# EdwardLiuyc/StaticMapping

Measured on AMD Instinct MI355X. Metric: scan-pair alignments/sec (120k-pt KITTI-64, 20 ICP iters), higher is better.
Workload: dtype f32/f64; 1 GPU; BASELINE config #2: IcpFast point-to-plane, 120k-pt synthetic Velodyne-64 scan pair vs CalculateNormals target (~21695 pts), exactly 20 iterations, rho 0.7; 512 distinct consecutive pairs of a synthetic drive (speed 6-10 m/s, yaw rate +-0.2 rad/s, seed 5), guess = previous pair's motion; pairs_per_gpu=512, distinct_pairs=512, target_points_mean=21695, nn_mode=grid, guess=extrapolated, split_after=2, parallelism=pairs round-robin over 1 GPU(s), one RCCL gather of poses, rccl_ranks=1

## Files before the change

### staticmapping_amd/csrc/icp_kernels.hip

```cpp
#include <type_traits>
#include "smhip_device.h"
#include "kd_median_tree.h"
#include "grid_lookup.h"

namespace smhip {

__device__ __forceinline__ bool xcd_block(int nblk, int npairs, int b_pair_base, int& pair, int& blk) {
  const int id = blockIdx.x;
  const int j = id >> 3;
  const int local = (j / nblk) * 8 + (id & 7);
  pair = b_pair_base + local;
  blk = j % nblk;
  return local < npairs;
}

__global__ __launch_bounds__(256) void tgt_reduce(IcpDev b) {
  const int pair = b.pair_base + blockIdx.y;
  const int nt = b.in[pair].nt;
  const float4* tp = b.tgt_p + (size_t)pair * b.nt_cap;
  double sx = 0, sy = 0, sz = 0;
  float mn[3] = {INFINITY, INFINITY, INFINITY}, mx[3] = {-INFINITY, -INFINITY, -INFINITY};
  const int chunk = (nt + gridDim.x - 1) / gridDim.x;
  const int lo = blockIdx.x * chunk, hi = min(nt, lo + chunk);
  for (int j = lo + threadIdx.x; j < hi; j += blockDim.x) {
// ... 1711 lines not shown
  if (threadIdx.x == 0) {
    const uint32_t active = (uint32_t)((nt + per - 1) / per);
    s_last = atomicAdd(&st->fallback_ticket, 1u) == active - 1u ? 1u : 0u;
  }
  __syncthreads();
  if (!s_last) return;
  __threadfence();
  for (int e = threadIdx.x; e < U; e += kNnThreads) {
    const int i = b.ulist[so + e];
    const unsigned long long key = __hip_atomic_load(&b.ukeys[so + e], __ATOMIC_RELAXED, __HIP_MEMORY_SCOPE_AGENT);
    const uint32_t dbits = (uint32_t)(key >> 32);
    b.d2[so + i] = __uint_as_float(dbits);
    st_match(b, so + i, (int)(uint32_t)(key & 0xffffffffu), 0.f);
    if (dbits < 0x7f800000u) atomicAdd(&b.hist[(size_t)pair * kHistBins + (dbits >> kHistShift)], 1u);
  }
  if (threadIdx.x == 0) st->fallback_ticket = 0;
}
__global__ __launch_bounds__(kNnThreads) void nn_fallback(IcpDev b) {
  const int pair = b.pair_base + blockIdx.y;
  PairState* st = &b.state[pair];
  if (st->done) return;
  __shared__ float4 s_t[kBruteTile];
  __shared__ uint32_t s_last;
  fallback_body(b, st, pair, (int)blockIdx.x, (int)gridDim.x, s_t, &s_last);
}


__device__ __forceinline__ int quantile_rank(uint32_t n_valid, float rho) {
  const double q = (double)rho;
  if (q >= 1.0) return (int)n_valid - 1;
  int k = (int)((double)n_valid * q);
  return min(k, (int)n_valid - 1);
}

__device__ __forceinline__ void find_quantile_bin_counts(const uint32_t* c, float rho, uint32_t* s_w, uint32_t* s_out) {
  constexpr int per = kHistBins / 256;
  uint32_t sum = 0;
#pragma unroll
  for (int k = 0; k < per; ++k) sum += c[k];
  uint32_t total;
  const uint32_t excl = block_excl_scan(sum, s_w, &total);
  if (threadIdx.x == 0) { s_out[0] = 0xffffffffu; s_out[1] = 0; s_out[2] = total; s_out[3] = 0; }
  __syncthreads();
  if (total > 0) {
    const uint32_t k = (uint32_t)quantile_rank(total, rho);
    if (excl <= k && k < excl + sum) {
      uint32_t run = excl;
#pragma unroll
      for (int t = 0; t < per; ++t) {
        if (k < run + c[t]) { s_out[0] = threadIdx.x * per + t; s_out[1] = run; s_out[3] = k; break; }
        run += c[t];
      }
    }
  }
  __syncthreads();
}
__device__ __forceinline__ void find_quantile_bin(const uint32_t* __restrict__ gh, float rho, uint32_t* s_w, uint32_t* s_out) {
  constexpr int per = kHistBins / 256;
  uint32_t c[per];
#pragma unroll
  for (int k = 0; k < per; ++k) c[k] = gh[threadIdx.x * per + k];
  find_quantile_bin_counts(c, rho, s_w, s_out);
}

__device__ __forceinline__ void validate_bounds(const IcpDev& b, PairState* st, int pair, uint32_t* s_w, uint32_t* s_q) {
  find_quantile_bin(b.hist + (size_t)pair * kHistBins, b.rho, s_w, s_q);
  if (threadIdx.x == 0) {
    const bool any = st->hard_count > 0;
    const bool below = (st->min_lb_key >> kHistShift) <= s_q[0];
    st->refine = (any && (b.exact_all || below || s_q[2] == 0)) ? 1 : 0;
    if (st->refine) st->refine_total += 1;
    st->spec_ok = (b.fused && st->band_lo > 0 && !st->refine && s_q[2] > 0 && (int)s_q[0] >= st->band_lo && (int)s_q[0] <= st->band_hi &&
                   st->deferred_count <= (uint32_t)kFusedListedMax) ? 1 : 0;
  }
}

__global__ __launch_bounds__(256) void nn_validate(IcpDev b) {
  const int pair = b.pair_base + blockIdx.x;
  PairState* st = &b.state[pair];
  if (st->done) return;
  __shared__ uint32_t s_w[17];
  __shared__ uint32_t s_q[4];
  validate_bounds(b, st, pair, s_w, s_q);
}

__global__ __launch_bounds__(kNnThreads) void nn_refine_one(IcpDev b) {
  const int pair = b.pair_base + blockIdx.x;
  PairState* st = &b.state[pair];
  if (st->done) return;
  __shared__ uint32_t s_w[17];
  __shared__ uint32_t s_q[4];
  __shared__ uint32_t s_hist[kHistBins];
  __shared__ float4 s_t[kBruteTile];
  __shared__ uint32_t s_last;
  validate_bounds(b, st, pair, s_w, s_q);
  __syncthreads();
  if (!st->refine) return;
  ring_body<true>(b, st, pair, 0, 1, s_hist);
  __syncthreads();
  fallback_body(b, st, pair, 0, 1, s_t, &s_last);
}

template <bool COUNT = true>
__device__ __forceinline__ void accumulate_terms_p(double px, double py, double pz, const float4 q4, const float4 n4, double* acc) {
  const double nx = n4.x, ny = n4.y, nz = n4.z;
  double J[6];
  J[0] = py * nz - pz * ny;
  J[1] = pz * nx - px * nz;
  J[2] = px * ny - py * nx;
  J[3] = nx; J[4] = ny; J[5] = nz;
  const double r = (px - (double)q4.x) * nx + (py - (double)q4.y) * ny + (pz - (double)q4.z) * nz;
  int c = 0;
#pragma unroll
  for (int a = 0; a < 6; ++a)
#pragma unroll
    for (int e = a; e < 6; ++e) acc[c++] += J[a] * J[e];
#pragma unroll
  for (int a = 0; a < 6; ++a) acc[21 + a] += J[a] * r;
  if (COUNT) acc[28] += 1.0;
}
__device__ __forceinline__ void accumulate_terms(const double* M, const float4 s4, const float4 q4, const float4 n4, double* acc) {
  double px, py, pz;
  transform_point(M, s4, px, py, pz);
  accumulate_terms_p(px, py, pz, q4, n4, acc);
}
template <int CTRL, int ROW_MASK>
__device__ __forceinline__ double dpp_or_zero(double v) {
  const int lo = __builtin_amdgcn_update_dpp(0, __double2loint(v), CTRL, ROW_MASK, 0xf, false);
  const int hi = __builtin_amdgcn_update_dpp(0, __double2hiint(v), CTRL, ROW_MASK, 0xf, false);
  return __hiloint2double(hi, lo);
}
__device__ __forceinline__ double wave_sum_to_last(double v) {
  v += dpp_or_zero<0x111, 0xf>(v);
  v += dpp_or_zero<0x112, 0xf>(v);
  v += dpp_or_zero<0x114, 0xf>(v);
  v += dpp_or_zero<0x118, 0xf>(v);
  v += dpp_or_zero<0x142, 0xa>(v);
  v += dpp_or_zero<0x143, 0xc>(v);
  return v;
}

__device__ __forceinline__ void block_reduce29(double* acc, double (*s_red)[29], double* s_out) {
  const int lane = threadIdx.x & 63, wave = threadIdx.x >> 6;
#pragma unroll
  for (int c = 0; c < 29; ++c) acc[c] = wave_sum_to_last(acc[c]);
  if (lane == 63)
#pragma unroll
    for (int c = 0; c < 29; ++c) s_red[wave][c] = acc[c];
  __syncthreads();
  if (threadIdx.x < 29) s_out[threadIdx.x] = ((s_red[0][threadIdx.x] + s_red[1][threadIdx.x]) + s_red[2][threadIdx.x]) + s_red[3][threadIdx.x];
  __syncthreads();
}

template <int ITEMS>
__device__ __forceinline__ void accumulate_block(const IcpDev& b, PairState* st, int pair, int blk, const double* Mc,
                                                 uint32_t* s_w, uint32_t* s_q, double (*s_red)[29], double* s_out) {
  const int ns = st->ns;
  const int base = blk * (kAccThreads * ITEMS);
  find_quantile_bin(b.hist + (size_t)pair * kHistBins, b.rho, s_w, s_q);
  const uint32_t qbin = s_q[0];
  double acc[29];
#pragma unroll
  for (int c = 0; c < 29; ++c) acc[c] = 0.0;
  const size_t so = (size_t)pair * b.ns_cap;
  const size_t to = (size_t)pair * b.nt_cap;
  const int seg = blk * (kAccThreads / 64) + (int)(threadIdx.x >> 6);
  const size_t segbase = (size_t)pair * 2 * b.bl_stride + (size_t)seg * (64 * ITEMS);
  int wcount = 0;
  int ic = min(base + (int)threadIdx.x, ns - 1);
  float d_1 = b.d2[so + ic];
  float4 s_1 = ld_src(b, so + ic);
  int j_1 = b.idx[so + ic];
  ic = min(base + kAccThreads + (int)threadIdx.x, ns - 1);
  float d_2 = b.d2[so + ic];
  float4 s_2 = ld_src(b, so + ic);
  int j_2 = b.idx[so + ic];
  float4 q_1 = make_float4(0, 0, 0, 0), n_1 = make_float4(0, 0, 0, 0);
  if ((__float_as_uint(d_1) >> kHistShift) < qbin) { q_1 = b.tq[to + max(j_1, 0)]; n_1 = b.tn[to + max(j_1, 0)]; }
#pragma unroll 2
  for (int it = 0; it < ITEMS; ++it) {
    const int i = base + it * kAccThreads + threadIdx.x;
    const float d = d_1;
    const float4 s4 = s_1;
    const float4 q4 = q_1, n4 = n_1;
    const int jm = j_1;
    d_1 = d_2; s_1 = s_2; j_1 = j_2;
    if (it + 1 < ITEMS && (__float_as_uint(d_1) >> kHistShift) < qbin) { q_1 = b.tq[to + max(j_1, 0)]; n_1 = b.tn[to + max(j_1, 0)]; }
    if (it + 2 < ITEMS) {
      ic = min(i + 2 * kAccThreads, ns - 1);
      d_2 = b.d2[so + ic];
      s_2 = ld_src(b, so + ic);
      j_2 = b.idx[so + ic];
    }
    bool boundary = false;
    if (i < ns) {
      const uint32_t key = __float_as_uint(d);
      if (key < 0x7f800000u) {
        const uint32_t bin = key >> kHistShift;
        if (bin < qbin) accumulate_terms(Mc, s4, q4, n4, acc);
        else boundary = bin == qbin;
      }
    }
    const unsigned long long bm = __ballot(boundary);
    if (boundary) {
      const size_t at = segbase + wcount + __popcll(bm & ((1ull << (threadIdx.x & 63)) - 1ull));
      b.rec_a[at] = make_float4(s4.x, s4.y, s4.z, d);
      b.rec_j[at] = jm;
    }
    wcount += (int)__popcll(bm);
  }
  if ((threadIdx.x & 63) == 0) b.gcount[(size_t)pair * b.seg_stride + seg] = (uint32_t)wcount;
  block_reduce29(acc, s_red, s_out);
  if (threadIdx.x < 29) b.partials[((size_t)pair * b.part_stride + blk) * kAccCols + threadIdx.x] = s_out[threadIdx.x];
}

template <int ITEMS>
__global__ __launch_bounds__(kAccThreads) void accumulate(IcpDev b, int nblk) {
  int pair, blk;
  if (!xcd_block(nblk, b.npairs, b.pair_base, pair, blk)) return;
  PairState* st = &b.state[pair];
  if (st->done) return;
  if (b.fused && st->spec_ok) return;
  if (blk * (kAccThreads * ITEMS) >= st->ns) return;
  double Mc[12];
#pragma unroll
  for (int k = 0; k < 12; ++k) Mc[k] = st->M[k];
  __shared__ uint32_t s_w[17];
  __shared__ uint32_t s_q[4];
  __shared__ double s_red[4][29];
  __shared__ double s_out[29];
  accumulate_block<ITEMS>(b, st, pair, blk, Mc, s_w, s_q, s_red, s_out);
}


__device__ __forceinline__ uint32_t rank_below(unsigned long long mask) {
  return __builtin_amdgcn_mbcnt_hi((uint32_t)(mask >> 32), __builtin_amdgcn_mbcnt_lo((uint32_t)mask, 0u));
}
__device__ __forceinline__ void emit_record(const IcpDev& b, size_t segbase, int& wcount, bool band, unsigned long long bm, const float4 s, float d, int j) {
  if (band) {
    const uint32_t k = rank_below(bm);
    char* __restrict__ ra = reinterpret_cast<char*>(b.rec_a + segbase + wcount);
    char* __restrict__ rj = reinterpret_cast<char*>(b.rec_j + segbase + wcount);
    *reinterpret_cast<float4*>(ra + k * 16u) = make_float4(s.x, s.y, s.z, d);
    *reinterpret_cast<int32_t*>(rj + k * 4u) = j;
  }
  wcount += (int)__popcll(bm);
}

template <int ITEMS, bool NABO = false, bool SHADOW = false>
__global__ __launch_bounds__(kNnThreads, NABO ? 4 : 1) void nn_certify_acc(IcpDev b, int nblk) {
  int pair, blk;
  if (!xcd_block(nblk, b.npairs, b.pair_base, pair, blk)) return;
  PairState* st = &b.state[pair];
  if (st->done) return;
  const int ns = st->ns;
  const int base = blk * (kNnThreads * ITEMS);
  if (base >= ns) return;
  double Mc[12];
#pragma unroll
  for (int k = 0; k < 12; ++k) Mc[k] = st->M[k];
  asm volatile("" : "+v"(Mc[3]), "+v"(Mc[7]), "+v"(Mc[11]));
  const Pot pot = {(float)st->pot_a, (float)st->pot_b, 0.f, 0.f};
  const int band_lo = st->band_lo, band_hi = st->band_hi;
  __shared__ uint32_t s_hist[kHistBins];
  __shared__ double s_red[4][29];
  __shared__ double s_out[29];
  for (int k = threadIdx.x; k < kHistBins; k += kNnThreads) s_hist[k] = 0;
  __syncthreads();
  const int lane = threadIdx.x & 63;
  const size_t so = (size_t)pair * b.ns_cap, to = (size_t)pair * b.nt_cap;
  const char* __restrict__ tqb = reinterpret_cast<const char*>(b.tq + to);
  const char* __restrict__ tnb = reinterpret_cast<const char*>(b.tn + to);
  const char* __restrict__ srcb = reinterpret_cast<const char*>(b.src3 + 3 * so);
  const char* __restrict__ lbb = reinterpret_cast<const char*>(b.lb + so);
  const char* __restrict__ idxb = reinterpret_cast<const char*>(b.idx + so);
  const char* __restrict__ mbb = reinterpret_cast<const char*>(b.mb + so);
  char* __restrict__ d2b = reinterpret_cast<char*>(b.d2 + so);
  auto ld_s = [&](int k) { const float3 v = *reinterpret_cast<const float3*>(srcb + __umul24((uint32_t)k, 12u)); return make_float4(v.x, v.y, v.z, 0.f); };
  auto ld_l = [&](int k) { return *reinterpret_cast<const float*>(lbb + (uint32_t)k * 4u); };
  auto ld_j = [&](int k) { return *reinterpret_cast<const int*>(idxb + (uint32_t)k * 4u); };
  auto ld_m = [&](int k) { return *reinterpret_cast<const uint32_t*>(mbb + (uint32_t)k * 4u); };
  auto ld_t = [&](const char* base, int j) { const float3 v = *reinterpret_cast<const float3*>(base + (uint32_t)max(j, 0) * 16u); return make_float4(v.x, v.y, v.z, 0.f); };
  auto st_d = [&](int k, float v) { *reinterpret_cast<float*>(d2b + (uint32_t)k * 4u) = v; };
  const float r_need = 0.9f * sqrtf(st->rcap2);
  uint32_t min_lb = 0xffffffffu;
  const int seg = blk * (kNnThreads / 64) + __builtin_amdgcn_readfirstlane((int)(threadIdx.x >> 6));
  const size_t recbase = (size_t)pair * 2 * b.bl_stride + (size_t)seg * (64 * ITEMS);
  char* __restrict__ dsegb = reinterpret_cast<char*>(b.dlist + (size_t)pair * b.dl_stride + (size_t)seg * (64 * ITEMS));
  int nrec = 0, ndef = 0, nkept = 0;
  uint32_t nabo_failed = 0;
  double acc[29];
#pragma unroll
  for (int c = 0; c < 29; ++c) acc[c] = 0.0;
  int ic = min(base + (int)threadIdx.x, ns - 1);
  float4 s_1 = ld_s(ic);
  float l_1, l_2;
  int j_1, j_2;
  uint32_t m_2 = 0;
  if (SHADOW) { const uint32_t m = ld_m(ic); l_1 = shadow_bound(m); j_1 = shadow_match(m); }
  else { l_1 = ld_l(ic); j_1 = ld_j(ic); }
  ic = min(base + kNnThreads + (int)threadIdx.x, ns - 1);
  float4 s_2 = ld_s(ic);
  if (SHADOW) { m_2 = ld_m(ic); l_2 = 0.f; j_2 = 0; }
  else { l_2 = ld_l(ic); j_2 = ld_j(ic); }
  float4 t_1 = ld_t(tqb, j_1);
  float4 n_1 = ld_t(tnb, j_1);
  auto round = [&](const int it, auto GATHER, auto STREAM) {
    const int i = base + it * kNnThreads + threadIdx.x;
    bool hard = false, fail = false, band = false;
    const float4 s = s_1;
    const float l = l_1;
    const int j = j_1;
    const float4 t = t_1, n = n_1;
    s_1 = s_2;
    if (SHADOW) { l_1 = shadow_bound(m_2); j_1 = shadow_match(m_2); }
    else { l_1 = l_2; j_1 = j_2; }
    if (GATHER.value) { t_1 = ld_t(tqb, j_1); n_1 = ld_t(tnb, j_1); }
    if (STREAM.value) {
      ic = min(i + 2 * kNnThreads, ns - 1);
      s_2 = ld_s(ic);
      if (SHADOW) m_2 = ld_m(ic);
      else { l_2 = ld_l(ic); j_2 = ld_j(ic); }
    }
    float d1 = 0.f;
    unsigned long long m_fail = 0, m_band = 0, m_hard = 0;
    if (NABO) {
      bool keep = false;
      if (i < ns) {
        double px, py, pz;
        transform_point(Mc, s, px, py, pz);
        const float qx = (float)px, qy = (float)py, qz = (float)pz;
        fail = true;
        const float Pn = pot_at(pot, norm3(s.x, s.y, s.z));
        if (isfinite(qx) && isfinite(qy) && isfinite(qz) && l > 0.f && j >= 0 &&
            l - Pn - 4.0e-7f * (l + Pn) - 1.3e-7f * (fabsf(qx) + fabsf(qy) + fabsf(qz)) > 0.f) {
          d1 = dist2(t, qx, qy, qz);
          st_d(i, d1);
          const int bin = (int)(__float_as_uint(d1) >> kHistShift);
          atomicAdd(&s_hist[bin], 1u);
          fail = false;
          if (bin < band_lo) { accumulate_terms_p<false>(px, py, pz, t, n, acc); keep = true; }
          else band = bin <= band_hi;
        }
      }
      nkept += (int)__popcll(__ballot(keep));
    } else {
      const auto B = [](bool p) { return (unsigned long long)__builtin_amdgcn_ballot_w64(p); };
      const auto P = [](unsigned long long m) { return (bool)__builtin_amdgcn_inverse_ballot_w64(m); };
      double px, py, pz;
      transform_point(Mc, s, px, py, pz);
      const float qx = (float)px, qy = (float)py, qz = (float)pz;
      const float Lp = bound_now(l, pot_at(pot, __builtin_amdgcn_sqrtf(fmaf(s.z, s.z, fmaf(s.y, s.y, s.x * s.x)))));
      const unsigned long long m_inr = B(i < ns);
      const unsigned long long m_pos = m_inr & B(Lp > 0.f);
      const unsigned long long m_has = B(l > 0.f) & B(j >= 0);
      d1 = dist2(t, qx, qy, qz);
      const unsigned long long m_ok = m_pos & m_has & B(d1 < Lp * Lp);
      const float zq = fmaf(qz, 0.f, fmaf(qy, 0.f, qx * 0.f));
      m_hard = m_pos & B(zq == 0.f) & ~m_has & B(l < 0.f) & B(Lp >= r_need);
      m_fail = m_inr & ~(m_ok | m_hard);
      const int bin = (int)(__float_as_uint(d1) >> kHistShift);
      const unsigned long long m_keep = m_ok & B(bin < band_lo);
      m_band = m_ok & ~m_keep & B(bin <= band_hi);
      nkept += (int)__popcll(m_keep);
      fail = P(m_fail); band = P(m_band); hard = P(m_hard);
      if (P(m_ok)) {
        st_d(i, d1);
        atomicAdd(&s_hist[bin], 1u);
      }
      if (P(m_keep)) accumulate_terms_p<false>(px, py, pz, t, n, acc);
      if (hard) {
        const float lb2 = Lp * Lp;
        st_d(i, lb2);
        atomicAdd(&s_hist[__float_as_uint(lb2) >> kHistShift], 1u);
        min_lb = min(min_lb, __float_as_uint(lb2));
      }
    }
    if (NABO) {
      if (fail) nabo_failed |= 1u << it;
      m_band = __ballot(band);
    } else {
      if (fail) *reinterpret_cast<int*>(dsegb + ((uint32_t)ndef + rank_below(m_fail)) * 4u) = i;
      ndef += (int)__popcll(m_fail);
    }
    emit_record(b, recbase, nrec, band, m_band, s, d1, j);
    const unsigned long long hm = m_hard;
    if (hm) {
      uint32_t basepos = 0;
      if (lane == 0) basepos = atomicAdd(&st->hard_count, (uint32_t)__popcll(hm));
      basepos = (uint32_t)__builtin_amdgcn_readlane((int)basepos, 0);
      if (hard) b.hlist[so + basepos + __popcll(hm & ((1ull << lane) - 1ull))] = i;
    }
  };
  static_assert(ITEMS >= 2, "the pipeline's last two rounds are written out");
#pragma unroll 2
  for (int it = 0; it < ITEMS - 2; ++it) round(it, std::true_type{}, std::true_type{});
  round(ITEMS - 2, std::true_type{}, std::false_type{});
  round(ITEMS - 1, std::false_type{}, std::false_type{});
  if (lane == 0) {
    b.gcount[(size_t)pair * b.seg_stride + seg] = (uint32_t)nrec;
    b.dcount[(size_t)pair * b.seg_stride + seg] = ndef;
  }
#pragma unroll
  for (int off = 32; off > 0; off >>= 1) min_lb = min(min_lb, (uint32_t)__shfl_xor((int)min_lb, off, 64));
  if (lane == 0 && min_lb != 0xffffffffu) atomicMin(&st->min_lb_key, min_lb);
  if (lane == 0) acc[28] = (double)nkept;
  block_reduce29(acc, s_red, s_out);
  if (threadIdx.x < 29) b.partials[((size_t)pair * b.part_stride + blk) * kAccCols + threadIdx.x] = s_out[threadIdx.x];
  if (NABO) nabo_list_append<ITEMS>(b, st, so, base, ns, nabo_failed, lane);
  uint32_t* gh = b.hist + (size_t)pair * kHistBins;
  for (int k = threadIdx.x; k < kHistBins; k += kNnThreads) {
    const uint32_t v = s_hist[k];
    if (v) atomicAdd(&gh[k], v);
  }
}

struct ListedCtx {
  const uint2* __restrict__ words; const uint32_t* __restrict__ cstart; const float4* __restrict__ tq;
  float ox, oy, oz, h, inv_h, r2cap;
  int nx, ny, nz, wx;
  uint32_t nt_last;
  bool have_prev;
  Pot pot;
};
__device__ __forceinline__ ListedCtx listed_ctx(const IcpDev& b, const PairState* st, int pair) {
  ListedCtx c;
  c.words = b.words + (size_t)pair * kMaxGridWords;
  c.cstart = b.cstart + (size_t)pair * (b.nt_cap + 1);
  c.tq = b.tq + (size_t)pair * b.nt_cap;
  c.ox = st->origin[0]; c.oy = st->origin[1]; c.oz = st->origin[2];
  c.h = st->h; c.inv_h = st->inv_h; c.r2cap = st->rcap2;
  c.nx = st->nx; c.ny = st->ny; c.nz = st->nz; c.wx = st->wx;
  c.nt_last = (uint32_t)max(st->nt - 1, 0);
  c.have_prev = st->iter > 0;
  c.pot = {(float)st->pot_a, (float)st->pot_b, 0.f, 0.f};
  return c;
}
__device__ __forceinline__ void listed_search_one(const IcpDev& b, const PairState* st, const ListedCtx& c, size_t so, int i, int sub, int L,
                                                  uint32_t* s_hist, uint32_t& min_lb, bool& hard, bool track_band, int band_lo, int band_hi,
                                                  bool& band, float4& srec, float& drec, int& jrec) {
  if (i < 0) {
    return;
  }
  const float4 s4 = ld_src(b, so + i);
  double px, py, pz;
  transform_point(st->M, s4, px, py, pz);
  const float qx = (float)px, qy = (float)py, qz = (float)pz;
  Best best = {INFINITY, -1, INFINITY};
  const bool finite = isfinite(qx) && isfinite(qy) && isfinite(qz);
  float R2 = c.r2cap;
  int jp = -1;
  if (finite) {
    if (c.have_prev) {
      jp = b.idx[so + i];
      if (jp >= 0) {
        double ux, uy, uz;
        transform_point(st->M_prev, s4, ux, uy, uz);
        const float ex = qx - (float)ux, ey = qy - (float)uy, ez = qz - (float)uz;
        R2 = search_radius2(c.r2cap, dist2(c.tq[jp], qx, qy, qz), search_margin(sqrtf(fmaf(ez, ez, fmaf(ey, ey, ex * ex)))));
      }
    }
    const float Rs = sqrtf(R2) * 1.0001f + 1.0e-3f * c.h;
    const int x0 = max(cell_coord(qx - Rs, c.ox, c.inv_h), 0), x1 = min(cell_coord(qx + Rs, c.ox, c.inv_h), c.nx - 1);
    const int y0 = max(cell_coord(qy - Rs, c.oy, c.inv_h), 0), y1 = min(cell_coord(qy + Rs, c.oy, c.inv_h), c.ny - 1);
    const int z0 = max(cell_coord(qz - Rs, c.oz, c.inv_h), 0), z1 = min(cell_coord(qz + Rs, c.oz, c.inv_h), c.nz - 1);
    const int nyr = y1 - y0 + 1;
    const int nrows = (x0 <= x1 && y0 <= y1 && z0 <= z1) ? nyr * (z1 - z0 + 1) : 0;
    const float slack = 2.0e-3f * c.h;
    const float inv_nyr = 1.0f / (float)max(nyr, 1);
    const uint32_t wa_i = (uint32_t)(x0 >> 5), wc_i = (uint32_t)(x1 >> 5);
    const uint32_t ma = (1u << (x0 & 31)) - 1u, mc = 0xffffffffu >> (31 - (x1 & 31));
    for (int rb = sub; rb < nrows; rb += 4 * L) {
      bool ok[4];
      uint2 wa[4], wc[4];
#pragma unroll
      for (int k = 0; k < 4; ++k) {
        const int r = rb + k * L, rr = min(r, nrows - 1);
        const int zr = (int)(((float)rr + 0.5f) * inv_nyr);
        const int z = z0 + zr, y = y0 + (rr - zr * nyr);
        const float zl = c.oz + (float)z * c.h, yl = c.oy + (float)y * c.h;
        const float dz = fmaxf(fmaxf(zl - qz, qz - (zl + c.h)) - slack, 0.f);
        const float dy = fmaxf(fmaxf(yl - qy, qy - (yl + c.h)) - slack, 0.f);
        ok[k] = r < nrows && !(fmaf(dy, dy, dz * dz) > R2);
        const int rowbase = (z * c.ny + y) * c.wx;
        wa[k] = c.words[rowbase + wa_i];
        wc[k] = c.words[rowbase + wc_i];
      }
      uint32_t j0[4], j1[4];
#pragma unroll
      for (int k = 0; k < 4; ++k) {
        const uint32_t sb = wa[k].y + __popc(wa[k].x & ma), se = wc[k].y + __popc(wc[k].x & mc);
        const bool has = ok[k] && se > sb;
        j0[k] = c.cstart[has ? sb : 0u];
        j1[k] = c.cstart[has ? se : 0u];
      }
      float4 t0[4];
#pragma unroll
      for (int k = 0; k < 4; ++k) t0[k] = c.tq[min(j0[k], c.nt_last)];
#pragma unroll
      for (int k = 0; k < 4; ++k) {
        if (j1[k] > j0[k]) {
          test_ascending_ru(t0[k], (int)j0[k], qx, qy, qz, best);
          for (uint32_t j = j0[k] + 1; j < j1[k]; j += 4) {
            const uint32_t e = j1[k] - 1u;
            const float4 a0 = c.tq[j], a1 = c.tq[min(j + 1u, e)], a2 = c.tq[min(j + 2u, e)], a3 = c.tq[min(j + 3u, e)];
            test_ascending_ru(a0, (int)j, qx, qy, qz, best);
            if (j + 1u <= e) test_ascending_ru(a1, (int)j + 1, qx, qy, qz, best);
            if (j + 2u <= e) test_ascending_ru(a2, (int)j + 2, qx, qy, qz, best);
            if (j + 3u <= e) test_ascending_ru(a3, (int)j + 3, qx, qy, qz, best);
          }
        }
      }
    }
  }
  for (int off = 1; off < L; off <<= 1) {
    const float od = __shfl_xor(best.d2, off, 64), os = __shfl_xor(best.s2, off, 64);
    const int oj = __shfl_xor(best.j, off, 64);
    best.s2 = fminf(fminf(best.s2, os), fmaxf(best.d2, od));
    if (od < best.d2 || (od == best.d2 && (unsigned)oj < (unsigned)best.j)) { best.d2 = od; best.j = oj; }
  }
  if (sub == 0) {
    float d2out = INFINITY, lbout = 0.f;
    int jout = -1;
    if (finite) {
      if (best.d2 <= R2) {
        d2out = best.d2;
        jout = best.j;
        lbout = sqrtf(fminf(best.s2, R2));
        if (track_band) {
          const int bin = (int)(__float_as_uint(d2out) >> kHistShift);
          band = bin >= band_lo && bin <= band_hi;
          srec = s4; drec = d2out; jrec = jout;
        }
      } else {
        d2out = R2;
        jout = best.j >= 0 ? best.j : jp;
        lbout = -sqrtf(R2);
        hard = true;
        min_lb = min(min_lb, __float_as_uint(R2));
      }
    }
    b.d2[so + i] = d2out;
    st_match(b, so + i, jout, with_pot(lbout, pot_at(c.pot, norm3(s4.x, s4.y, s4.z))));
    const uint32_t key = __float_as_uint(d2out);
    if (key < 0x7f800000u) atomicAdd(&s_hist[key >> kHistShift], 1u);
  }
}
__device__ __forceinline__ int listed_lanes_log2(int count, int budget = kListedBlocks * kNnThreads) {
  int L = 1, logL = 0;
  while (L < 16 && 2 * L * count <= budget) { L *= 2; ++logL; }
  return logL;
}
__device__ __forceinline__ void listed_append_hard(const IcpDev& b, PairState* st, size_t so, bool hard, int i, int lane) {
  const unsigned long long hm = __ballot(hard);
  if (hm) {
    uint32_t basepos = 0;
    if (lane == 0) basepos = atomicAdd(&st->hard_count, (uint32_t)__popcll(hm));
    basepos = (uint32_t)__builtin_amdgcn_readlane((int)basepos, 0);
    if (hard) b.hlist[so + basepos + __popcll(hm & ((1ull << lane) - 1ull))] = i;
  }
// ... 155 lines not shown
    const int e = chunk * qpb + ql;
    int i = -1;
    if (e < count) {
      const int32_t* __restrict__ dl = b.dlist + (size_t)pair * b.dl_stride;
      int sg = 0;
      for (int step = top; step > 0; step >>= 1) { const int cand = sg + step; sg = s_off[cand] <= (uint32_t)e ? cand : sg; }
      i = dl[(size_t)sg * (64 * kCertifyItems) + (e - (int)s_off[sg])];
    }
    bool hard = false, band = false;
    float4 srec = make_float4(0.f, 0.f, 0.f, 0.f);
    float drec = 0.f;
    int jrec = -1;
    listed_search_one(b, st, c, so, i, sub, L, s_hist, min_lb, hard, band_lo > 0, band_lo, band_hi, band, srec, drec, jrec);
    listed_append_hard(b, st, so, hard, i, lane);
    if (band_lo > 0) {
      const unsigned long long bm = __ballot(band);
      uint32_t* wc = s_wc[item & 1];
      if (lane == 0) wc[wave] = (uint32_t)__popcll(bm);
      __syncthreads();
      uint32_t before = 0, all = 0;
#pragma unroll
      for (int w2 = 0; w2 < kNnThreads / 64; ++w2) { const uint32_t n2 = wc[w2]; before += w2 < wave ? n2 : 0u; all += n2; }
      if (band) {
        const size_t at = (size_t)pair * 2 * b.bl_stride + (size_t)b.bl_stride + (size_t)chunk * qpb + before + __popcll(bm & ((1ull << lane) - 1ull));
        b.rec_a[at] = make_float4(srec.x, srec.y, srec.z, drec);
        b.rec_j[at] = jrec;
      }
      if (threadIdx.x == 0) b.gcount[(size_t)pair * b.seg_stride + nseg0 + chunk] = all;
    }
  }
  if (cur >= 0) flush();
}

__device__ __forceinline__ void listed_sums_block(const IcpDev& b, PairState* st, int pair, int item, uint32_t* s_off, double (*s_red)[29], double* s_out) {
  const int ns = st->ns;
  const int nblk = (ns + kNnThreads * kCertifyItems - 1) / (kNnThreads * kCertifyItems);
  const int nseg0 = nblk * (kNnThreads / 64);
  const int32_t* dc = b.dcount + (size_t)pair * b.seg_stride;
  const int32_t* dl = b.dlist + (size_t)pair * b.dl_stride;
  int top = 1;
  while (2 * top < nseg0) top *= 2;
  for (int x = threadIdx.x; x < 2 * top; x += kAccThreads) s_off[x] = x < nseg0 ? (uint32_t)dc[x] : 0xffffffffu;
  const int nl = dc[nseg0];
  __syncthreads();
  const int band_lo = st->band_lo;
  const size_t so = (size_t)pair * b.ns_cap, to = (size_t)pair * b.nt_cap;
  double acc[29];
#pragma unroll
  for (int c = 0; c < 29; ++c) acc[c] = 0.0;
  constexpr int kL = 4;
  const int e_end = min(nl, (item + 1) * kListedSumChunk);
  for (int e0 = item * kListedSumChunk + (int)threadIdx.x; e0 < e_end; e0 += kL * kAccThreads) {
    int sg[kL], ii[kL], jj[kL];
    float dd[kL];
    float4 s4[kL], q4[kL], n4[kL];
#pragma unroll
    for (int k = 0; k < kL; ++k) sg[k] = 0;
    for (int step = top; step > 0; step >>= 1) {
#pragma unroll
      for (int k = 0; k < kL; ++k) {
        const int cand = sg[k] + step;
        sg[k] = s_off[cand] <= (uint32_t)min(e0 + kAccThreads * k, e_end - 1) ? cand : sg[k];
      }
    }
#pragma unroll
    for (int k = 0; k < kL; ++k) ii[k] = dl[(size_t)sg[k] * (64 * kCertifyItems) + (min(e0 + kAccThreads * k, e_end - 1) - (int)s_off[sg[k]])];
#pragma unroll
    for (int k = 0; k < kL; ++k) { s4[k] = ld_src(b, so + ii[k]); jj[k] = b.idx[so + ii[k]]; dd[k] = b.d2[so + ii[k]]; }
#pragma unroll
    for (int k = 0; k < kL; ++k) { q4[k] = b.tq[to + max(jj[k], 0)]; n4[k] = b.tn[to + max(jj[k], 0)]; }
#pragma unroll
    for (int k = 0; k < kL; ++k) {
      const uint32_t key = __float_as_uint(dd[k]);
      if (e0 + kAccThreads * k < e_end && jj[k] >= 0 && key < 0x7f800000u && (int)(key >> kHistShift) < band_lo)
        accumulate_terms(st->M, s4[k], q4[k], n4[k], acc);
    }
  }
  block_reduce29(acc, s_red, s_out);
  if (threadIdx.x < 29) b.partials[((size_t)pair * b.part_stride + nblk + item) * kAccCols + threadIdx.x] = s_out[threadIdx.x];
}

template <int ITEMS>
__global__ __launch_bounds__(kAccThreads) void iteration_sums(IcpDev b) {
  __shared__ uint32_t s_w[17];
  __shared__ uint32_t s_q[4];
  __shared__ double s_red[4][29];
  __shared__ double s_out[29];
  __shared__ uint32_t s_plan[kListedMaxPairs / 8 + 1];
  __shared__ uint32_t s_off[2 * kFinalizeMaxSeg];
  const int x = (int)blockIdx.x & 7, lw = (int)blockIdx.x >> 3, nlw = (int)gridDim.x >> 3;
  const int npx = (b.npairs - x + 7) >> 3;
  {
    uint32_t mine = 0;
    if ((int)threadIdx.x < npx) {
      const PairState* st = &b.state[b.pair_base + (int)threadIdx.x * 8 + x];
      if (!st->done) {
        if (st->spec_ok) mine = (st->deferred_count + (uint32_t)kListedSumChunk - 1u) / (uint32_t)kListedSumChunk;
        else mine = (uint32_t)((st->ns + kAccThreads * ITEMS - 1) / (kAccThreads * ITEMS));
      }
    }
    uint32_t total;
    const uint32_t o = block_excl_scan(mine, s_w, &total);
    if ((int)threadIdx.x < npx) s_plan[threadIdx.x] = o;
    if (threadIdx.x == 0) s_plan[npx] = total;
    __syncthreads();
  }
  const int nitems = (int)s_plan[npx];
  int lo = 0;
  for (int item = lw; item < nitems; item += nlw) {
    while (s_plan[lo + 1] <= (uint32_t)item) ++lo;
    const int pair = b.pair_base + lo * 8 + x;
    PairState* st = &b.state[pair];
    const int k = item - (int)s_plan[lo];
    if (st->spec_ok) {
      listed_sums_block(b, st, pair, k, s_off, s_red, s_out);
    } else {
      double Mc[12];
#pragma unroll
      for (int c = 0; c < 12; ++c) Mc[c] = st->M[c];
      accumulate_block<ITEMS>(b, st, pair, k, Mc, s_w, s_q, s_red, s_out);
    }
    __syncthreads();
  }
}

__global__ __launch_bounds__(kAccThreads) void nabo_validate(IcpDev b) {
  const int pair = b.pair_base + (int)blockIdx.x;
  PairState* st = &b.state[pair];
  if (st->done) return;
  __shared__ uint32_t s_w[17];
  __shared__ uint32_t s_q[4];
  find_quantile_bin(b.hist + (size_t)pair * kHistBins, b.rho, s_w, s_q);
  if (threadIdx.x == 0) {
    const int band_lo = st->band_lo, band_hi = st->band_hi;
    st->spec_ok = (band_lo > 0 && s_q[2] > 0 && (int)s_q[0] >= band_lo && (int)s_q[0] <= band_hi) ? 1 : 0;
  }
}
__global__ __launch_bounds__(kAccThreads) void accumulate_listed(IcpDev b) {
  const int pair = b.pair_base + (int)blockIdx.y, blk = (int)blockIdx.x;
  PairState* st = &b.state[pair];
  if (st->done) return;
  __shared__ double s_red[4][29];
  __shared__ double s_out[29];
  const int ns = st->ns;
  const int nblk0 = (ns + kNnThreads * kCertifyItems - 1) / (kNnThreads * kCertifyItems);
  const int nseg0 = nblk0 * (kNnThreads / 64);
  int cls_first[5];
  cls_first[0] = 0;
#pragma unroll
  for (int c = 0; c < 4; ++c) cls_first[c + 1] = cls_first[c] + (int)st->nabo_count[c];
  const int total = cls_first[4];
  constexpr int kWaves = kNaboAccBlocks * (kAccThreads / 64);
  const int lane = threadIdx.x & 63, wave = blk * (kAccThreads / 64) + (int)(threadIdx.x >> 6);
  const int share = (total + kWaves - 1) / kWaves;
  const int e0 = wave * share, e1 = min(total, e0 + share);
  if (blk != 0 && blk * (kAccThreads / 64) * share >= total) {
    if (lane == 0) b.gcount[(size_t)pair * b.seg_stride + nseg0 + wave] = 0u;
    if (threadIdx.x < 29) b.partials[((size_t)pair * b.part_stride + nblk0 + blk) * kAccCols + threadIdx.x] = 0.0;
    return;
  }
  if (!st->spec_ok) return;
  const int band_lo = st->band_lo, band_hi = st->band_hi;
  const size_t so = (size_t)pair * b.ns_cap, to = (size_t)pair * b.nt_cap;
  const int seg_len1 = b.bl_stride / kWaves;
  const size_t segbase = (size_t)pair * 2 * b.bl_stride + (size_t)b.bl_stride + (size_t)wave * seg_len1;
  double Mc[12];
#pragma unroll
  for (int k = 0; k < 12; ++k) Mc[k] = st->M[k];
  double acc[29];
#pragma unroll
  for (int c = 0; c < 29; ++c) acc[c] = 0.0;
  int wcount = 0;
  auto entry = [&](int e) -> int {
    const int c = e < cls_first[1] ? 0 : (e < cls_first[2] ? 1 : (e < cls_first[3] ? 2 : 3));
    const int f = c == 0 ? cls_first[0] : (c == 1 ? cls_first[1] : (c == 2 ? cls_first[2] : cls_first[3]));
    return *nabo_list_slot(b, so, c, (uint32_t)(e - f));
  };
  constexpr int kU = 2;
  for (int eb = e0; eb < e1; eb += 64 * kU) {
    int i[kU], jm[kU];
    float d[kU];
    float4 s4[kU], q4[kU], n4[kU];
    bool live[kU], below[kU], rec[kU];
#pragma unroll
    for (int u = 0; u < kU; ++u) { live[u] = eb + 64 * u + lane < e1; i[u] = live[u] ? entry(eb + 64 * u + lane) : 0; }
#pragma unroll
    for (int u = 0; u < kU; ++u) { d[u] = b.d2[so + i[u]]; jm[u] = b.idx[so + i[u]]; s4[u] = ld_src(b, so + i[u]); }
#pragma unroll
    for (int u = 0; u < kU; ++u) {
      const uint32_t key = __float_as_uint(d[u]);
      const int bin = (int)(key >> kHistShift);
      const bool valid = live[u] && key < 0x7f800000u && jm[u] >= 0;
      below[u] = valid && bin < band_lo;
      rec[u] = valid && bin >= band_lo && bin <= band_hi;
      if (below[u]) { q4[u] = b.tq[to + jm[u]]; n4[u] = b.tn[to + jm[u]]; }
    }
#pragma unroll
    for (int u = 0; u < kU; ++u) {
      if (below[u]) accumulate_terms(Mc, s4[u], q4[u], n4[u], acc);
      const unsigned long long bm = __ballot(rec[u]);
      if (rec[u]) {
        const size_t at = segbase + wcount + __popcll(bm & ((1ull << lane) - 1ull));
        b.rec_a[at] = make_float4(s4[u].x, s4[u].y, s4[u].z, d[u]);
        b.rec_j[at] = jm[u];
      }
      wcount += (int)__popcll(bm);
    }
  }
  if (lane == 0) b.gcount[(size_t)pair * b.seg_stride + nseg0 + wave] = (uint32_t)wcount;
  block_reduce29(acc, s_red, s_out);
  if (threadIdx.x < 29) b.partials[((size_t)pair * b.part_stride + nblk0 + blk) * kAccCols + threadIdx.x] = s_out[threadIdx.x];
}

__device__ __noinline__ void jacobi_eig6(double* A, double* V, double* w) {
  for (int i = 0; i < 6; ++i) for (int j = 0; j < 6; ++j) V[6 * i + j] = (i == j) ? 1.0 : 0.0;
  for (int sweep = 0; sweep < 60; ++sweep) {
    double off = 0;
    for (int i = 0; i < 6; ++i) for (int j = i + 1; j < 6; ++j) off += A[6 * i + j] * A[6 * i + j];
    if (off < 1e-300) break;
    for (int p = 0; p < 6; ++p)
      for (int q = p + 1; q < 6; ++q) {
        const double apq = A[6 * p + q];
        if (fabs(apq) < 1e-300) continue;
        const double theta = (A[6 * q + q] - A[6 * p + p]) / (2.0 * apq);
        const double t = (theta >= 0 ? 1.0 : -1.0) / (fabs(theta) + sqrt(theta * theta + 1.0));
        const double c = 1.0 / sqrt(t * t + 1.0), s = t * c;
        for (int k = 0; k < 6; ++k) { const double akp = A[6 * k + p], akq = A[6 * k + q]; A[6 * k + p] = c * akp - s * akq; A[6 * k + q] = s * akp + c * akq; }
        for (int k = 0; k < 6; ++k) { const double apk = A[6 * p + k], aqk = A[6 * q + k]; A[6 * p + k] = c * apk - s * aqk; A[6 * q + k] = s * apk + c * aqk; }
        for (int k = 0; k < 6; ++k) { const double vkp = V[6 * k + p], vkq = V[6 * k + q]; V[6 * k + p] = c * vkp - s * vkq; V[6 * k + q] = s * vkp + c * vkq; }
      }
  }
  for (int i = 0; i < 6; ++i) w[i] = A[6 * i + i];
}

__device__ __forceinline__ void solve6(const double* A, const double* rhs, double* x) {
  double L[36];
  double dmax = 0;
#pragma unroll
  for (int i = 0; i < 6; ++i) dmax = fmax(dmax, fabs(A[6 * i + i]));
  bool ok = dmax > 0 && isfinite(dmax);
#pragma unroll
  for (int i = 0; i < 6; ++i)
#pragma unroll
    for (int j = 0; j <= i; ++j) {
      double s = A[6 * i + j];
#pragma unroll
      for (int k = 0; k < j; ++k) s -= L[6 * i + k] * L[6 * j + k];
      if (i == j) {
        ok = ok && (s > 1e-13 * dmax);
        L[6 * i + i] = sqrt(s);
      } else {
        L[6 * i + j] = s / L[6 * j + j];
      }
    }
  if (ok) {
    double y[6];
#pragma unroll
    for (int i = 0; i < 6; ++i) {
      double s = rhs[i];
#pragma unroll
      for (int k = 0; k < i; ++k) s -= L[6 * i + k] * y[k];
      y[i] = s / L[6 * i + i];
    }
#pragma unroll
    for (int i = 5; i >= 0; --i) {
      double s = y[i];
#pragma unroll
      for (int k = i + 1; k < 6; ++k) s -= L[6 * k + i] * x[k];
      x[i] = s / L[6 * i + i];
    }
    return;
  }
  double E[36], V[36], w[6];
#pragma unroll
  for (int i = 0; i < 36; ++i) E[i] = A[i];
  jacobi_eig6(E, V, w);
  double wmax = 0;
  for (int i = 0; i < 6; ++i) wmax = fmax(wmax, fabs(w[i]));
  const double thresh = 2.220446049250313e-16 * 6 * wmax;
  for (int i = 0; i < 6; ++i) x[i] = 0;
  for (int k = 0; k < 6; ++k) {
    if (!(fabs(w[k]) > thresh)) continue;
    double c = 0;
    for (int i = 0; i < 6; ++i) c += V[6 * i + k] * rhs[i];
    c /= w[k];
    for (int i = 0; i < 6; ++i) x[i] += c * V[6 * i + k];
  }
}

__device__ void quat_from_rot(const double* T, double* q) {
  const double r00 = T[0], r01 = T[1], r02 = T[2], r10 = T[4], r11 = T[5], r12 = T[6], r20 = T[8], r21 = T[9], r22 = T[10];
  const double tr = r00 + r11 + r22;
  if (tr > 0) {
    const double s = sqrt(tr + 1.0) * 2;
    q[0] = 0.25 * s; q[1] = (r21 - r12) / s; q[2] = (r02 - r20) / s; q[3] = (r10 - r01) / s;
  } else if (r00 >= r11 && r00 >= r22) {
    const double s = sqrt(1.0 + r00 - r11 - r22) * 2;
    q[0] = (r21 - r12) / s; q[1] = 0.25 * s; q[2] = (r01 + r10) / s; q[3] = (r02 + r20) / s;
  } else if (r11 >= r22) {
    const double s = sqrt(1.0 + r11 - r00 - r22) * 2;
    q[0] = (r02 - r20) / s; q[1] = (r01 + r10) / s; q[2] = 0.25 * s; q[3] = (r12 + r21) / s;
  } else {
    const double s = sqrt(1.0 + r22 - r00 - r11) * 2;
    q[0] = (r10 - r01) / s; q[1] = (r02 + r20) / s; q[2] = (r12 + r21) / s; q[3] = 0.25 * s;
  }
}

__device__ double quat_angular_distance(const double* a, const double* c) {
  const double w = a[0] * c[0] + a[1] * c[1] + a[2] * c[2] + a[3] * c[3];
  const double x = -a[0] * c[1] + a[1] * c[0] - a[2] * c[3] + a[3] * c[2];
  const double y = -a[0] * c[2] + a[2] * c[0] - a[3] * c[1] + a[1] * c[3];
  const double z = -a[0] * c[3] + a[3] * c[0] - a[1] * c[2] + a[2] * c[1];
  return 2.0 * atan2(sqrt(x * x + y * y + z * z), fabs(w));
}

struct TailOpts {
  float cap_factor, ball_radius, band_gain, band_pad;
  int32_t fused, early_exit, max_iteration;
  uint32_t* search_hist;
  uint32_t* done_count;
};
template <class B>
__device__ __forceinline__ uint32_t finalize_tail(const B& b, PairState* st, int pair, const double* s_tot, uint32_t n_valid, uint32_t limit_key,
                                                  bool fusedm, int ns, bool publish) {
  st->fallback_total += st->unresolved_count;
  st->unresolved_count = 0;
  st->hard_total += st->hard_count;
  st->hard_count = 0;
  {
    const uint32_t walked = st->nabo_count[0] + st->nabo_count[1] + st->nabo_count[2] + st->nabo_count[3];
    const uint32_t searched = st->iter == 0 ? (uint32_t)ns : (walked ? walked : (st->deferred_count ? st->deferred_count : (uint32_t)ns));
    st->searched_total += searched;
    if (publish && st->iter < kSearchHist) b.search_hist[(size_t)pair * kSearchHist + st->iter] = searched;
    for (int c = 0; c < 4; ++c) st->nabo_count[c] = 0;
  }
  const uint32_t n_listed = st->deferred_count;
  st->deferred_count = 0;
  st->min_lb_key = 0xffffffffu;
  st->refine = 0;
  {
    const float lim = sqrtf(__uint_as_float(limit_key));
    float rc = fminf(fmaxf(b.cap_factor * lim, 0.05f), b.ball_radius);
    if (!(n_valid > 0)) rc = b.ball_radius;
    st->rcap2 = rc * rc;
  }
  {
    const uint32_t prev = st->limit_key;
    int lo = 0, hi = -1;
    if (n_valid > 0 && prev != 0u && limit_key != 0u) {
      const double x = (double)limit_key;
      const double w = fmax((double)b.band_gain * fabs(x - (double)prev), (double)b.band_pad * 1048576.0);
      const double l = x - w, u = x + w;
      if (l >= 1048576.0 && u < 2139095040.0) { lo = (int)((uint32_t)l >> kHistShift); hi = (int)((uint32_t)u >> kHistShift); }
      if (hi - lo > 2) { lo = 0; hi = -1; }
      if (b.fused && n_listed > (uint32_t)kFusedListedMax) { lo = 0; hi = -1; }
    }
    st->band_lo = lo; st->band_hi = hi;
    if (fusedm) st->spec_hits += 1;
    st->spec_ok = 0;
  }
// ... 399 lines not shown
```

Before: 26390 alignments/s.

## Split normal-equation accumulators across lane pairs, deepen NN prefetch pipeline, bitmap-sort nabo list

The 27 upper-triangle normal-equation sums are split between even and odd lanes, with DPP swaps exchanging Jacobian terms, so each lane holds 14 double accumulators instead of 29. Launch bounds for nn_certify_acc go to 4 waves per SIMD. The per-round software pipeline now runs four rounds deep with staggered normal, point and word loads. The nabo accumulate pass rebuilds per-wave index bitmaps in LDS so entries are visited in source-index order rather than list order. Together these aim to cut register pressure, raise occupancy and improve gather locality, but every lane now does the accumulate work including masked ones, and the bitmap pass rescans the whole nabo list once per block.

```diff
diff --git a/staticmapping_amd/csrc/icp_kernels.hip b/staticmapping_amd/csrc/icp_kernels.hip
--- a/staticmapping_amd/csrc/icp_kernels.hip
+++ b/staticmapping_amd/csrc/icp_kernels.hip
@@ -1887,6 +1887,69 @@
   __syncthreads();
 }
 
+__host__ __device__ constexpr int pair_slot_a(int k) { return (int)((0x10020420420420ull >> (4 * k)) & 15); }
+__host__ __device__ constexpr int pair_slot_e(int k) { return (int)((0x43442531666420ull >> (4 * k)) & 15); }
+__host__ __device__ constexpr int pair_slot_col(int k, int odd) {
+  const int a = (pair_slot_a(k) + odd) % 6, e6 = pair_slot_e(k);
+  if (e6 == 6) return 21 + a;
+  const int e = (e6 + odd) % 6, lo = a < e ? a : e, hi = a < e ? e : a;
+  return lo * 6 - lo * (lo - 1) / 2 + (hi - lo);
+}
+constexpr int kPairSlots = 14;
+__host__ __device__ constexpr bool pair_col_is_even(int c) {
+  for (int k = 0; k < kPairSlots; ++k) if (pair_slot_col(k, 0) == c) return true;
+  return false;
+}
+constexpr bool pair_slots_cover_each_column_once() {
+  int n[27] = {};
+  for (int k = 0; k < kPairSlots; ++k) {
+    n[pair_slot_col(k, 0)] += 1;
+    if (!pair_col_is_even(pair_slot_col(k, 1))) n[pair_slot_col(k, 1)] += 1;
+  }
+  for (int c = 0; c < 27; ++c) if (n[c] != 1) return false;
+  return true;
+}
+static_assert(pair_slots_cover_each_column_once(), "every column of the row from exactly one slot of one parity (block_reduce_pair_sums)");
+__device__ __forceinline__ void accumulate_terms_pair(double px, double py, double pz, const float4 q4, const float4 n4, bool keep, bool odd, double* acc) {
+  const double nx = n4.x, ny = n4.y, nz = n4.z;
+  const auto z = [keep](double x) { return keep ? x : 0.0; };
+  const auto sw = [](double x) {
+    const int lo = __double2loint(x), hi = __double2hiint(x);
+    return __hiloint2double(__builtin_amdgcn_update_dpp(hi, hi, 0xb1, 0xf, 0xf, false), __builtin_amdgcn_update_dpp(lo, lo, 0xb1, 0xf, 0xf, false));
+  };
+  const double j0 = z(py * nz - pz * ny), j1 = z(pz * nx - px * nz), j2 = z(px * ny - py * nx), j3 = z(nx), j4 = z(ny), j5 = z(nz);
+  const double r = z((px - (double)q4.x) * nx + (py - (double)q4.y) * ny + (pz - (double)q4.z) * nz);
+  {
+    const double own[7] = {odd ? j1 : j0, odd ? j2 : j1, odd ? j3 : j2, odd ? j4 : j3, odd ? j5 : j4, odd ? j0 : j5, r};
+#pragma unroll
+    for (int k = 0; k < kPairSlots; ++k) acc[k] += own[pair_slot_a(k)] * own[pair_slot_e(k)];
+  }
+  {
+    const double par[7] = {sw(odd ? j0 : j1), sw(odd ? j1 : j2), sw(odd ? j2 : j3), sw(odd ? j3 : j4), sw(odd ? j4 : j5), sw(odd ? j5 : j0), sw(r)};
+#pragma unroll
+    for (int k = 0; k < kPairSlots; ++k) acc[k] += par[pair_slot_a(k)] * par[pair_slot_e(k)];
+  }
+#pragma unroll
+  for (int k = 0; k < kPairSlots; ++k) asm volatile("" : "+v"(acc[k]));
+}
+__device__ __forceinline__ void block_reduce_pair_sums(const double* acc, bool odd, int nkept, double (*s_red)[29], double* s_out) {
+  const int lane = threadIdx.x & 63, wave = threadIdx.x >> 6;
+#pragma unroll
+  for (int k = 0; k < kPairSlots; ++k) {
+    const int ce = pair_slot_col(k, 0), co = pair_slot_col(k, 1);
+    const double e = wave_sum_to_last(odd ? 0.0 : acc[k]);
+    if (lane == 63) s_red[wave][ce] = e;
+    if (!pair_col_is_even(co)) {
+      const double o = wave_sum_to_last(odd ? acc[k] : 0.0);
+      if (lane == 63) s_red[wave][co] = o;
+    }
+  }
+  if (lane == 63) { s_red[wave][27] = 0.0; s_red[wave][28] = (double)nkept; }
+  __syncthreads();
+  if (threadIdx.x < 29) s_out[threadIdx.x] = ((s_red[0][threadIdx.x] + s_red[1][threadIdx.x]) + s_red[2][threadIdx.x]) + s_red[3][threadIdx.x];
+  __syncthreads();
+}
+
 template <int ITEMS>
 __device__ __forceinline__ void accumulate_block(const IcpDev& b, PairState* st, int pair, int blk, const double* Mc,
                                                  uint32_t* s_w, uint32_t* s_q, double (*s_red)[29], double* s_out) {
@@ -1983,7 +2046,7 @@
 }
 
 template <int ITEMS, bool NABO = false, bool SHADOW = false>
-__global__ __launch_bounds__(kNnThreads, NABO ? 4 : 1) void nn_certify_acc(IcpDev b, int nblk) {
+__global__ __launch_bounds__(kNnThreads, 4) void nn_certify_acc(IcpDev b, int nblk) {
   int pair, blk;
   if (!xcd_block(nblk, b.npairs, b.pair_base, pair, blk)) return;
   PairState* st = &b.state[pair];
@@ -2024,46 +2087,47 @@
   char* __restrict__ dsegb = reinterpret_cast<char*>(b.dlist + (size_t)pair * b.dl_stride + (size_t)seg * (64 * ITEMS));
   int nrec = 0, ndef = 0, nkept = 0;
   uint32_t nabo_failed = 0;
-  double acc[29];
-#pragma unroll
-  for (int c = 0; c < 29; ++c) acc[c] = 0.0;
-  int ic = min(base + (int)threadIdx.x, ns - 1);
-  float4 s_1 = ld_s(ic);
-  float l_1, l_2;
-  int j_1, j_2;
-  uint32_t m_2 = 0;
-  if (SHADOW) { const uint32_t m = ld_m(ic); l_1 = shadow_bound(m); j_1 = shadow_match(m); }
-  else { l_1 = ld_l(ic); j_1 = ld_j(ic); }
-  ic = min(base + kNnThreads + (int)threadIdx.x, ns - 1);
-  float4 s_2 = ld_s(ic);
-  if (SHADOW) { m_2 = ld_m(ic); l_2 = 0.f; j_2 = 0; }
-  else { l_2 = ld_l(ic); j_2 = ld_j(ic); }
-  float4 t_1 = ld_t(tqb, j_1);
-  float4 n_1 = ld_t(tnb, j_1);
-  auto round = [&](const int it, auto GATHER, auto STREAM) {
-    const int i = base + it * kNnThreads + threadIdx.x;
+  const bool odd = (lane & 1) != 0;
+  double acc[kPairSlots];
+#pragma unroll
+  for (int c = 0; c < kPairSlots; ++c) acc[c] = 0.0;
+  float4 s_r[4], t_r[4], n_r[2];
+  float l_r[4];
+  int j_r[4];
+  uint32_t m_r[4];
+  auto ld_w = [&](int slot, int k) {
+    if (SHADOW) m_r[slot] = ld_m(k);
+    else { l_r[slot] = ld_l(k); j_r[slot] = ld_j(k); }
+  };
+  auto id_of = [&](int slot) { return SHADOW ? shadow_match(m_r[slot]) : j_r[slot]; };
+#pragma unroll
+  for (int k = 0; k < 4; ++k) ld_w(k, min(base + k * kNnThreads + (int)threadIdx.x, ns - 1));
+  s_r[0] = ld_s(min(base + (int)threadIdx.x, ns - 1));
+  s_r[1] = ld_s(min(base + kNnThreads + (int)threadIdx.x, ns - 1));
+  t_r[0] = ld_t(tqb, id_of(0));
+  n_r[0] = ld_t(tnb, id_of(0));
+  t_r[1] = ld_t(tqb, id_of(1));
+  auto round = [&](const int i0, const int r0, auto PH, auto NORMAL, auto POINT, auto WORD) {
+    constexpr int ph = decltype(PH)::value;
+    const int it = r0 + ph;
+    const int i = i0 + ph * kNnThreads;
     bool hard = false, fail = false, band = false;
-    const float4 s = s_1;
-    const float l = l_1;
-    const int j = j_1;
-    const float4 t = t_1, n = n_1;
-    s_1 = s_2;
-    if (SHADOW) { l_1 = shadow_bound(m_2); j_1 = shadow_match(m_2); }
-    else { l_1 = l_2; j_1 = j_2; }
-    if (GATHER.value) { t_1 = ld_t(tqb, j_1); n_1 = ld_t(tnb, j_1); }
-    if (STREAM.value) {
-      ic = min(i + 2 * kNnThreads, ns - 1);
-      s_2 = ld_s(ic);
-      if (SHADOW) m_2 = ld_m(ic);
-      else { l_2 = ld_l(ic); j_2 = ld_j(ic); }
-    }
+    const float l = SHADOW ? shadow_bound(m_r[ph]) : l_r[ph];
+    const int j = id_of(ph);
+    if (NORMAL.value) n_r[(ph + 1) & 1] = ld_t(tnb, id_of((ph + 1) & 3));
+    if (POINT.value) {
+      t_r[(ph + 2) & 3] = ld_t(tqb, id_of((ph + 2) & 3));
+      s_r[(ph + 2) & 3] = ld_s(min(i + 2 * kNnThreads, ns - 1));
+    }
+    if (WORD.value) ld_w(ph, min(i + 4 * kNnThreads, ns - 1));
+    const float4 s = s_r[ph], t = t_r[ph], n = n_r[ph & 1];
     float d1 = 0.f;
     unsigned long long m_fail = 0, m_band = 0, m_hard = 0;
     if (NABO) {
       bool keep = false;
+      double px, py, pz;
+      transform_point(Mc, s, px, py, pz);
       if (i < ns) {
-        double px, py, pz;
-        transform_point(Mc, s, px, py, pz);
         const float qx = (float)px, qy = (float)py, qz = (float)pz;
         fail = true;
         const float Pn = pot_at(pot, norm3(s.x, s.y, s.z));
@@ -2074,10 +2138,11 @@
           const int bin = (int)(__float_as_uint(d1) >> kHistShift);
           atomicAdd(&s_hist[bin], 1u);
           fail = false;
-          if (bin < band_lo) { accumulate_terms_p<false>(px, py, pz, t, n, acc); keep = true; }
-          else band = bin <= band_hi;
+          keep = bin < band_lo;
+          band = !keep && bin <= band_hi;
         }
       }
+      accumulate_terms_pair(px, py, pz, t, n, keep, odd, acc);
       nkept += (int)__popcll(__ballot(keep));
     } else {
       const auto B = [](bool p) { return (unsigned long long)__builtin_amdgcn_ballot_w64(p); };
@@ -2103,7 +2168,7 @@
         st_d(i, d1);
         atomicAdd(&s_hist[bin], 1u);
       }
-      if (P(m_keep)) accumulate_terms_p<false>(px, py, pz, t, n, acc);
+      accumulate_terms_pair(px, py, pz, t, n, P(m_keep), odd, acc);
       if (hard) {
         const float lb2 = Lp * Lp;
         st_d(i, lb2);
@@ -2124,14 +2189,26 @@
       uint32_t basepos = 0;
       if (lane == 0) basepos = atomicAdd(&st->hard_count, (uint32_t)__popcll(hm));
       basepos = (uint32_t)__builtin_amdgcn_readlane((int)basepos, 0);
-      if (hard) b.hlist[so + basepos + __popcll(hm & ((1ull << lane) - 1ull))] = i;
+      if (hard) b.hlist[so + basepos + rank_below(hm)] = i;
     }
   };
-  static_assert(ITEMS >= 2, "the pipeline's last two rounds are written out");
-#pragma unroll 2
-  for (int it = 0; it < ITEMS - 2; ++it) round(it, std::true_type{}, std::true_type{});
-  round(ITEMS - 2, std::true_type{}, std::false_type{});
-  round(ITEMS - 1, std::false_type{}, std::false_type{});
+  static_assert(ITEMS % 4 == 0 && ITEMS >= 8, "four rounds per trip; the pipeline's last four rounds are written out");
+  using Y = std::true_type; using N = std::false_type;
+  using P0 = std::integral_constant<int, 0>; using P1 = std::integral_constant<int, 1>; using P2 = std::integral_constant<int, 2>; using P3 = std::integral_constant<int, 3>;
+  int i0 = base + (int)threadIdx.x;
+#pragma unroll 1
+  for (int r0 = 0; r0 < ITEMS - 4; r0 += 4) {
+    asm volatile("" : "+v"(i0));
+    round(i0, r0, P0{}, Y{}, Y{}, Y{});
+    round(i0, r0, P1{}, Y{}, Y{}, Y{});
+    round(i0, r0, P2{}, Y{}, Y{}, Y{});
+    round(i0, r0, P3{}, Y{}, Y{}, Y{});
+    i0 += 4 * kNnThreads;
+  }
+  round(i0, ITEMS - 4, P0{}, Y{}, Y{}, N{});
+  round(i0, ITEMS - 4, P1{}, Y{}, Y{}, N{});
+  round(i0, ITEMS - 4, P2{}, Y{}, N{}, N{});
+  round(i0, ITEMS - 4, P3{}, N{}, N{}, N{});
   if (lane == 0) {
     b.gcount[(size_t)pair * b.seg_stride + seg] = (uint32_t)nrec;
     b.dcount[(size_t)pair * b.seg_stride + seg] = ndef;
@@ -2139,8 +2216,7 @@
 #pragma unroll
   for (int off = 32; off > 0; off >>= 1) min_lb = min(min_lb, (uint32_t)__shfl_xor((int)min_lb, off, 64));
   if (lane == 0 && min_lb != 0xffffffffu) atomicMin(&st->min_lb_key, min_lb);
-  if (lane == 0) acc[28] = (double)nkept;
-  block_reduce29(acc, s_red, s_out);
+  block_reduce_pair_sums(acc, odd, nkept, s_red, s_out);
   if (threadIdx.x < 29) b.partials[((size_t)pair * b.part_stride + blk) * kAccCols + threadIdx.x] = s_out[threadIdx.x];
   if (NABO) nabo_list_append<ITEMS>(b, st, so, base, ns, nabo_failed, lane);
   uint32_t* gh = b.hist + (size_t)pair * kHistBins;
@@ -2602,9 +2678,12 @@
   const int total = cls_first[4];
   constexpr int kWaves = kNaboAccBlocks * (kAccThreads / 64);
   const int lane = threadIdx.x & 63, wave = blk * (kAccThreads / 64) + (int)(threadIdx.x >> 6);
-  const int share = (total + kWaves - 1) / kWaves;
-  const int e0 = wave * share, e1 = min(total, e0 + share);
-  if (blk != 0 && blk * (kAccThreads / 64) * share >= total) {
+  constexpr int kRange = 4096, kWords = kRange / 32;
+  __shared__ uint32_t s_bits[kAccThreads / 64][kWords];
+  __shared__ uint32_t s_pre[kAccThreads / 64][kWords];
+  static_assert(kAccThreads / 64 == 4, "four bitmaps per workgroup");
+  const int range = (ns + kWaves - 1) / kWaves;
+  if (total == 0) {
     if (lane == 0) b.gcount[(size_t)pair * b.seg_stride + nseg0 + wave] = 0u;
     if (threadIdx.x < 29) b.partials[((size_t)pair * b.part_stride + nblk0 + blk) * kAccCols + threadIdx.x] = 0.0;
     return;
@@ -2627,35 +2706,79 @@
     return *nabo_list_slot(b, so, c, (uint32_t)(e - f));
   };
   constexpr int kU = 2;
-  for (int eb = e0; eb < e1; eb += 64 * kU) {
-    int i[kU], jm[kU];
-    float d[kU];
-    float4 s4[kU], q4[kU], n4[kU];
-    bool live[kU], below[kU], rec[kU];
-#pragma unroll
-    for (int u = 0; u < kU; ++u) { live[u] = eb + 64 * u + lane < e1; i[u] = live[u] ? entry(eb + 64 * u + lane) : 0; }
-#pragma unroll
-    for (int u = 0; u < kU; ++u) { d[u] = b.d2[so + i[u]]; jm[u] = b.idx[so + i[u]]; s4[u] = ld_src(b, so + i[u]); }
-#pragma unroll
-    for (int u = 0; u < kU; ++u) {
-      const uint32_t key = __float_as_uint(d[u]);
-      const int bin = (int)(key >> kHistShift);
-      const bool valid = live[u] && key < 0x7f800000u && jm[u] >= 0;
-      below[u] = valid && bin < band_lo;
-      rec[u] = valid && bin >= band_lo && bin <= band_hi;
-      if (below[u]) { q4[u] = b.tq[to + jm[u]]; n4[u] = b.tn[to + jm[u]]; }
-    }
-#pragma unroll
-    for (int u = 0; u < kU; ++u) {
-      if (below[u]) accumulate_terms(Mc, s4[u], q4[u], n4[u], acc);
-      const unsigned long long bm = __ballot(rec[u]);
-      if (rec[u]) {
-        const size_t at = segbase + wcount + __popcll(bm & ((1ull << lane) - 1ull));
-        b.rec_a[at] = make_float4(s4[u].x, s4[u].y, s4[u].z, d[u]);
-        b.rec_j[at] = jm[u];
-      }
-      wcount += (int)__popcll(bm);
-    }
+  const int wv = (int)(threadIdx.x >> 6);
+  for (int p0 = 0; p0 < range; p0 += kRange) {
+    for (int k = threadIdx.x; k < (kAccThreads / 64) * kWords; k += kAccThreads) (&s_bits[0][0])[k] = 0u;
+    __syncthreads();
+    constexpr int kS = 32;
+    for (int eb = 0; eb < total; eb += kAccThreads * kS) {
+      int iq[kS];
+#pragma unroll
+      for (int s = 0; s < kS; ++s) { const int e = eb + s * kAccThreads + (int)threadIdx.x; iq[s] = e < total ? entry(e) : -1; }
+#pragma unroll
+      for (int s = 0; s < kS; ++s) {
+        const int rel = iq[s] - blk * (kAccThreads / 64) * range;
+        if (iq[s] >= 0 && rel >= 0 && rel < (kAccThreads / 64) * range) {
+          int wq = rel >= 2 * range ? 2 : 0;
+          wq += rel - wq * range >= range ? 1 : 0;
+          const int off = rel - wq * range - p0;
+          if (off >= 0 && off < kRange) atomicOr(&s_bits[wq][off >> 5], 1u << (off & 31));
+        }
+      }
+    }
+    __syncthreads();
+    static_assert(kWords == 128, "two words per lane");
+    const int ca = __popc(s_bits[wv][2 * lane]), cb = __popc(s_bits[wv][2 * lane + 1]);
+    int incl = ca + cb;
+#pragma unroll
+    for (int off = 1; off < 64; off <<= 1) { const int v = __shfl_up(incl, off, 64); if (lane >= off) incl += v; }
+    s_pre[wv][2 * lane] = (uint32_t)(incl - ca - cb);
+    s_pre[wv][2 * lane + 1] = (uint32_t)(incl - cb);
+    const int e1 = __shfl(incl, 63, 64);
+    __syncthreads();
+    for (int eb = 0; eb < e1; eb += 64 * kU) {
+      int i[kU], jm[kU];
+      float d[kU];
+      float4 s4[kU], q4[kU], n4[kU];
+      bool live[kU], below[kU], rec[kU];
+#pragma unroll
+      for (int u = 0; u < kU; ++u) {
+        const int r = eb + 64 * u + lane;
+        live[u] = r < e1;
+        i[u] = 0;
+        if (live[u]) {
+          int wd = 0;
+#pragma unroll
+          for (int step = kWords / 2; step > 0; step >>= 1) if ((int)s_pre[wv][wd + step] <= r) wd += step;
+          uint32_t w = s_bits[wv][wd];
+          for (int t = r - (int)s_pre[wv][wd]; t > 0; --t) w &= w - 1u;
+          i[u] = wave * range + p0 + wd * 32 + (__ffs(w) - 1);
+        }
+      }
+#pragma unroll
+      for (int u = 0; u < kU; ++u) { d[u] = b.d2[so + i[u]]; jm[u] = b.idx[so + i[u]]; s4[u] = ld_src(b, so + i[u]); }
+#pragma unroll
+      for (int u = 0; u < kU; ++u) {
+        const uint32_t key = __float_as_uint(d[u]);
+        const int bin = (int)(key >> kHistShift);
+        const bool valid = live[u] && key < 0x7f800000u && jm[u] >= 0;
+        below[u] = valid && bin < band_lo;
+        rec[u] = valid && bin >= band_lo && bin <= band_hi;
+        if (below[u]) { q4[u] = b.tq[to + jm[u]]; n4[u] = b.tn[to + jm[u]]; }
+      }
+#pragma unroll
+      for (int u = 0; u < kU; ++u) {
+        if (below[u]) accumulate_terms(Mc, s4[u], q4[u], n4[u], acc);
+        const unsigned long long bm = __ballot(rec[u]);
+        if (rec[u]) {
+          const size_t at = segbase + wcount + __popcll(bm & ((1ull << lane) - 1ull));
+          b.rec_a[at] = make_float4(s4[u].x, s4[u].y, s4[u].z, d[u]);
+          b.rec_j[at] = jm[u];
+        }
+        wcount += (int)__popcll(bm);
+      }
+    }
+    __syncthreads();
   }
   if (lane == 0) b.gcount[(size_t)pair * b.seg_stride + nseg0 + wave] = (uint32_t)wcount;
   block_reduce29(acc, s_red, s_out);
```

Result: faster. 27320 alignments/s, median of 6 (+3.5%).
